# 4paradigm/OpenEmbedding

Hardware: NVIDIA H100
Metric: samples/sec (whole job, device-timed, max over ranks) deepfm Criteo dim 64 (higher is better)
Workload: dtype bf16

## Files before the change

openembedding_b200/csrc/cuda/gemm_wgmma.cu:

```cuda
#include <cuda.h>
#include <cuda_bf16.h>
#include <cuda_runtime.h>
#include "pdl.cuh"
#include <stdint.h>
#include <stdio.h>
#include <stdlib.h>
#include <string.h>

#include <string>
#include <vector>
#include <algorithm>

namespace {

constexpr int BM = 128, BK = 64;
constexpr int A_BYTES = BM * BK * 2;
template <int BN> constexpr int stages_for() { return BN == 64 ? 4 : 3; }
constexpr int NUM_CONSUMER_WARPS = 8;
constexpr int PRODUCER_WARP = NUM_CONSUMER_WARPS;
constexpr int NUM_THREADS = 32 * (NUM_CONSUMER_WARPS + 1);

enum EpiMode : int { EPI_FWD = 0, EPI_DX = 1, EPI_DW = 2, EPI_DX_FM = 3 };

struct GemmEpi {
// ... 34 lines not shown
    for (uint32_t it = 0; it < (1u << 24); ++it)
        if (mbar_try(b, parity)) return true;
    atomicAdd(&g_pipeline_timeouts, 1u);
    return false;
}
__device__ __forceinline__ void tma_load_2d(void* smem_dst, const CUtensorMap* map, uint64_t* bar, int c0, int c1) {
    asm volatile("cp.async.bulk.tensor.2d.shared::cluster.global.mbarrier::complete_tx::bytes [%0], [%1, {%3, %4}], [%2];"
                 ::"r"(smem_u32(smem_dst)), "l"(map), "r"(smem_u32(bar)), "r"(c0), "r"(c1) : "memory");
}
__device__ __forceinline__ void tma_load_2d_mc(void* smem_dst, const CUtensorMap* map, uint64_t* bar, int c0, int c1, uint16_t mask) {
    asm volatile("cp.async.bulk.tensor.2d.shared::cluster.global.mbarrier::complete_tx::bytes.multicast::cluster [%0], [%1, {%4, %5}], [%2], %3;"
                 ::"r"(smem_u32(smem_dst)), "l"(map), "r"(smem_u32(bar)), "h"(mask), "r"(c0), "r"(c1) : "memory");
}
__device__ __forceinline__ void cluster_sync_all() {
    asm volatile("barrier.cluster.arrive.release.aligned;" ::: "memory");
    asm volatile("barrier.cluster.wait.acquire.aligned;" ::: "memory");
}
__device__ __forceinline__ void named_bar_sync(int id, int threads) {
    asm volatile("bar.sync %0, %1;" ::"r"(id), "r"(threads) : "memory");
}

__device__ __forceinline__ uint64_t gmma_desc(uint32_t smem_addr, uint32_t lbo_bytes) {
    uint64_t d = 0;
    d |= (uint64_t)((smem_addr & 0x3FFFFu) >> 4);
    d |= (uint64_t)((lbo_bytes >> 4) & 0x3FFFu) << 16;
    d |= (uint64_t)(1024 >> 4) << 32;
    d |= (uint64_t)1 << 62;
    return d;
}
__device__ __forceinline__ void wgmma_fence() { asm volatile("wgmma.fence.sync.aligned;" ::: "memory"); }
__device__ __forceinline__ void wgmma_commit() { asm volatile("wgmma.commit_group.sync.aligned;" ::: "memory"); }
template <int N>
__device__ __forceinline__ void wgmma_wait() { asm volatile("wgmma.wait_group.sync.aligned %0;" ::"n"(N) : "memory"); }
template <int R>
__device__ __forceinline__ void acc_fence(float (&d)[R]) {
#pragma unroll
    for (int i = 0; i < R; ++i) asm volatile("" : "+f"(d[i])::"memory");
}

template <int TRANS>
__device__ __forceinline__ void wgmma_n64(float (&d)[32], uint64_t da, uint64_t db, uint32_t scale_d) {
    asm volatile("{\n\t.reg .pred p;\n\tsetp.ne.b32 p, %34, 0;\n\t"
                 "wgmma.mma_async.sync.aligned.m64n64k16.f32.bf16.bf16 {"
                 "%0, %1, %2, %3, %4, %5, %6, %7, %8, %9, %10, %11, %12, %13, %14, %15, "
                 "%16, %17, %18, %19, %20, %21, %22, %23, %24, %25, %26, %27, %28, %29, %30, %31"
                 "}, %32, %33, p, 1, 1, %35, %35;\n\t}"
                 : "+f"(d[0]), "+f"(d[1]), "+f"(d[2]), "+f"(d[3]), "+f"(d[4]), "+f"(d[5]), "+f"(d[6]), "+f"(d[7]),
                   "+f"(d[8]), "+f"(d[9]), "+f"(d[10]), "+f"(d[11]), "+f"(d[12]), "+f"(d[13]), "+f"(d[14]), "+f"(d[15]),
                   "+f"(d[16]), "+f"(d[17]), "+f"(d[18]), "+f"(d[19]), "+f"(d[20]), "+f"(d[21]), "+f"(d[22]), "+f"(d[23]),
                   "+f"(d[24]), "+f"(d[25]), "+f"(d[26]), "+f"(d[27]), "+f"(d[28]), "+f"(d[29]), "+f"(d[30]), "+f"(d[31])
                 : "l"(da), "l"(db), "r"(scale_d), "n"(TRANS));
}
template <int TRANS>
__device__ __forceinline__ void wgmma_n128(float (&d)[64], uint64_t da, uint64_t db, uint32_t scale_d) {
    asm volatile("{\n\t.reg .pred p;\n\tsetp.ne.b32 p, %66, 0;\n\t"
                 "wgmma.mma_async.sync.aligned.m64n128k16.f32.bf16.bf16 {"
                 "%0, %1, %2, %3, %4, %5, %6, %7, %8, %9, %10, %11, %12, %13, %14, %15, "
                 "%16, %17, %18, %19, %20, %21, %22, %23, %24, %25, %26, %27, %28, %29, %30, %31, "
                 "%32, %33, %34, %35, %36, %37, %38, %39, %40, %41, %42, %43, %44, %45, %46, %47, "
                 "%48, %49, %50, %51, %52, %53, %54, %55, %56, %57, %58, %59, %60, %61, %62, %63"
                 "}, %64, %65, p, 1, 1, %67, %67;\n\t}"
                 : "+f"(d[0]), "+f"(d[1]), "+f"(d[2]), "+f"(d[3]), "+f"(d[4]), "+f"(d[5]), "+f"(d[6]), "+f"(d[7]),
                   "+f"(d[8]), "+f"(d[9]), "+f"(d[10]), "+f"(d[11]), "+f"(d[12]), "+f"(d[13]), "+f"(d[14]), "+f"(d[15]),
                   "+f"(d[16]), "+f"(d[17]), "+f"(d[18]), "+f"(d[19]), "+f"(d[20]), "+f"(d[21]), "+f"(d[22]), "+f"(d[23]),
                   "+f"(d[24]), "+f"(d[25]), "+f"(d[26]), "+f"(d[27]), "+f"(d[28]), "+f"(d[29]), "+f"(d[30]), "+f"(d[31]),
                   "+f"(d[32]), "+f"(d[33]), "+f"(d[34]), "+f"(d[35]), "+f"(d[36]), "+f"(d[37]), "+f"(d[38]), "+f"(d[39]),
                   "+f"(d[40]), "+f"(d[41]), "+f"(d[42]), "+f"(d[43]), "+f"(d[44]), "+f"(d[45]), "+f"(d[46]), "+f"(d[47]),
                   "+f"(d[48]), "+f"(d[49]), "+f"(d[50]), "+f"(d[51]), "+f"(d[52]), "+f"(d[53]), "+f"(d[54]), "+f"(d[55]),
                   "+f"(d[56]), "+f"(d[57]), "+f"(d[58]), "+f"(d[59]), "+f"(d[60]), "+f"(d[61]), "+f"(d[62]), "+f"(d[63])
                 : "l"(da), "l"(db), "r"(scale_d), "n"(TRANS));
}
template <int BN, int TRANS>
__device__ __forceinline__ void wgmma_stage(float (&acc)[BN / 2], uint32_t a0, uint32_t b0, int g, bool first) {
#pragma unroll
    for (int k = 0; k < BK / 16; ++k) {
        const uint64_t da = TRANS ? gmma_desc(a0 + g * 8192 + k * 2048, 8192) : gmma_desc(a0 + g * 8192 + k * 32, 16);
        const uint64_t db = TRANS ? gmma_desc(b0 + k * 2048, 8192) : gmma_desc(b0 + k * 32, 16);
        const uint32_t sd = (first && k == 0) ? 0u : 1u;
        if constexpr (BN == 64) wgmma_n64<TRANS>(acc, da, db, sd);
        else wgmma_n128<TRANS>(acc, da, db, sd);
    }
}

template <int BN>
__device__ __forceinline__ void mma_tile(float (&acc)[BN / 2], const uint8_t* sA, const uint8_t* sB, uint64_t* full,
                                         uint64_t* empty, int stages, uint32_t kiter, int nkb, bool mn_major, int g,
                                         int C) {
    constexpr int B_BYTES = BN * BK * 2;
    const int lane = threadIdx.x & 31;
#pragma unroll
    for (int j = 0; j < BN / 2; ++j) acc[j] = 0.f;
    auto release = [&](uint32_t it) {
        const int s = it % stages;
        if (C > 1) { if (lane < C) mbar_arrive_cluster(&empty[s], (uint32_t)lane); }
        else if (lane == 0) mbar_arrive(&empty[s]);
    };
    for (int i = 0; i < nkb; ++i) {
        const uint32_t it = kiter + i;
        const int s = it % stages;
        mbar_wait(&full[s], (it / stages) & 1u);
        const uint32_t a0 = smem_u32(sA + s * A_BYTES), b0 = smem_u32(sB + s * B_BYTES);
        wgmma_fence();
        if (mn_major) wgmma_stage<BN, 1>(acc, a0, b0, g, i == 0);
        else wgmma_stage<BN, 0>(acc, a0, b0, g, i == 0);
        wgmma_commit();
        if (i > 0) {
            wgmma_wait<1>();
            acc_fence(acc);
            release(it - 1);
        }
    }
    wgmma_wait<0>();
    acc_fence(acc);
    if (nkb > 0) release(kiter + nkb - 1);
}

template <int BN>
__device__ __forceinline__ void epilogue_tile(const GemmEpi& E, float (&acc)[BN / 2], int m_blk, int n_blk, int g,
                                              uint8_t* stage, int qstride, const CUtensorMap* tO, const CUtensorMap* tT) {
    const int t = threadIdx.x & 127, w = t >> 5, l = t & 31;
    const bool f32out = (E.mode == EPI_DW || E.mode == EPI_DX_FM);
    const int q = 2 * g + (w >> 1);
    uint8_t* wstage = stage + q * qstride;
    uint8_t* tstage = wstage + BN * 128;
#pragma unroll
    for (int i = 0; i < 2; ++i) {
        const int qrow = (w & 1) * 16 + (l >> 2) + 8 * i;
        const int row = m_blk * BM + q * 32 + qrow;
        const bool rv = row < E.M;
        const float dl = (E.mode == EPI_DX_FM && rv && n_blk * BN < E.fm_cols) ? E.dlogit[row] : 0.f;
#pragma unroll
        for (int j = 0; j < BN / 8; ++j) {
            const int c = 8 * j + 2 * (l & 3);
            const int n = n_blk * BN + c;
            float x[2] = {acc[4 * j + 2 * i], acc[4 * j + 2 * i + 1]};
            if (E.mode == EPI_FWD) {
#pragma unroll
                for (int u = 0; u < 2; ++u) {
                    if (E.relu) x[u] = fmaxf(x[u], 0.f);
                    if (n + u == E.ones_col) x[u] = 1.f;
                    if (n + u >= E.N) x[u] = 0.f;
                }
            } else if (E.mode == EPI_DX) {
                float2 mk = make_float2(0.f, 0.f);
                if (rv && n < E.N) mk = __bfloat1622float2(*reinterpret_cast<const __nv_bfloat162*>(E.mask + (size_t)row * E.ldmask + n));
                const float mv[2] = {mk.x, mk.y};
#pragma unroll
                for (int u = 0; u < 2; ++u)
                    if (!rv || !(mv[u] > 0.f) || n + u == E.ones_col || n + u >= E.N) x[u] = 0.f;
            } else if (E.mode == EPI_DX_FM && rv && n < E.fm_cols) {
                const float2 e2 = *reinterpret_cast<const float2*>(E.emb + (size_t)row * E.ldemb + n);
                const float* sb = E.S + (size_t)row * E.D;
                x[0] += dl * (sb[n % E.D] - e2.x);
                x[1] += dl * (sb[(n + 1) % E.D] - e2.y);
            }
            if (f32out) {
                const int cc = c & 31;
                *reinterpret_cast<float2*>(wstage + (c >> 5) * 4096 + qrow * 128 + ((((cc >> 2) ^ (qrow & 7))) << 4) + (cc & 3) * 4) =
                    make_float2(x[0], x[1]);
            } else {
                const int cc = c & 63;
                *reinterpret_cast<__nv_bfloat162*>(wstage + (c >> 6) * 4096 + qrow * 128 + ((((cc >> 3) ^ (qrow & 7))) << 4) + (cc & 7) * 2) =
                    __floats2bfloat162_rn(x[0], x[1]);
                if (E.outT) {
                    *reinterpret_cast<__nv_bfloat16*>(tstage + c * 64 + qrow * 2) = __float2bfloat16_rn(x[0]);
                    *reinterpret_cast<__nv_bfloat16*>(tstage + (c + 1) * 64 + qrow * 2) = __float2bfloat16_rn(x[1]);
                }
            }
        }
    }
    asm volatile("fence.proxy.async.shared::cta;" ::: "memory");
    named_bar_sync(2 + g, 128);
    if (t == 0) {
        if (E.fm_cols != -7) {
#pragma unroll 1
            for (int qq = 2 * g; qq < 2 * g + 2; ++qq) {
                const int row0 = m_blk * BM + qq * 32;
                uint8_t* ws = stage + qq * qstride;
                if (f32out) {
#pragma unroll 1
                    for (int h = 0; h < BN / 32; ++h) {
                        const int n0 = n_blk * BN + 32 * h;
                        if (E.mode == EPI_DW)
                            asm volatile("cp.reduce.async.bulk.tensor.2d.global.shared::cta.add.tile.bulk_group [%0, {%2, %3}], [%1];"
                                         ::"l"(tO), "r"(smem_u32(ws + h * 4096)), "r"(n0), "r"(row0) : "memory");
                        else
                            asm volatile("cp.async.bulk.tensor.2d.global.shared::cta.bulk_group [%0, {%2, %3}], [%1];"
                                         ::"l"(tO), "r"(smem_u32(ws + h * 4096)), "r"(n0), "r"(row0) : "memory");
                    }
                } else {
#pragma unroll 1
                    for (int h = 0; h < BN / 64; ++h)
                        asm volatile("cp.async.bulk.tensor.2d.global.shared::cta.bulk_group [%0, {%2, %3}], [%1];"
                                     ::"l"(tO), "r"(smem_u32(ws + h * 4096)), "r"(n_blk * BN + 64 * h), "r"(row0) : "memory");
                    if (E.outT)
                        asm volatile("cp.async.bulk.tensor.2d.global.shared::cta.bulk_group [%0, {%2, %3}], [%1];"
                                     ::"l"(tT), "r"(smem_u32(ws + BN * 128)), "r"(row0), "r"(n_blk * BN) : "memory");
                }
            }
        }
        asm volatile("cp.async.bulk.commit_group;" ::: "memory");
    }
}

template <int BN>
__global__ void __launch_bounds__(NUM_THREADS, 2)
exb_gemm_wgmma_kernel(const __grid_constant__ CUtensorMap tmA, const __grid_constant__ CUtensorMap tmB,
                      const __grid_constant__ CUtensorMap tmO, const __grid_constant__ CUtensorMap tmT,
                      GemmEpi E, int num_k_blocks, int k_blocks_per_split) {
    static_assert(BN == 64 || BN == 128, "tile width");
    constexpr int STAGES = stages_for<BN>();
    constexpr int B_BYTES = BN * BK * 2;
    constexpr int QSTAGE = BN * 128 + BN * 64;
    static_assert(4 * QSTAGE <= STAGES * (A_BYTES + B_BYTES), "epilogue staging aliases the stage memory");
    extern __shared__ __align__(1024) uint8_t smem_raw[];
    uint8_t* smem = smem_raw + ((1024u - (smem_u32(smem_raw) & 1023u)) & 1023u);
    uint8_t* sA = smem;
    uint8_t* sB = smem + STAGES * A_BYTES;
    uint64_t* full = reinterpret_cast<uint64_t*>(sB + STAGES * B_BYTES);
    uint64_t* empty = full + STAGES;

    exb::pdl_trigger();
    const int warp = threadIdx.x >> 5, lane = threadIdx.x & 31;
    const int m_blk = E.swap ? blockIdx.y : blockIdx.x, n_blk = E.swap ? blockIdx.x : blockIdx.y;
    const bool dbg = E.dbg != nullptr && blockIdx.x == 0 && blockIdx.y == 0 && blockIdx.z == 0;
#define GSTAMP(i) do { if (dbg) { unsigned long long _t; asm volatile("mov.u64 %0, %%globaltimer;" : "=l"(_t)); E.dbg[i] = _t; } } while (0)
    if (threadIdx.x == 0) GSTAMP(0);
    const int kb0 = blockIdx.z * k_blocks_per_split;
    const int kb1 = min(num_k_blocks, kb0 + k_blocks_per_split);
    const int nkb = kb1 - kb0;
    const int C = E.mc > 1 ? E.mc : 1;
    uint32_t crank = 0;
    if (C > 1) asm volatile("mov.u32 %0, %%cluster_ctarank;" : "=r"(crank));
    const uint16_t cmask = (uint16_t)((1u << C) - 1u);

    if (threadIdx.x == 0) {
        for (int i = 0; i < STAGES; ++i) { mbar_init(&full[i], 1); mbar_init(&empty[i], (uint32_t)(NUM_CONSUMER_WARPS * C)); }
        asm volatile("fence.mbarrier_init.release.cluster;" ::: "memory");
        asm volatile("prefetch.tensormap [%0];" ::"l"(&tmA) : "memory");
        asm volatile("prefetch.tensormap [%0];" ::"l"(&tmB) : "memory");
    }
    __syncthreads();
    if (C > 1) cluster_sync_all();
    exb::pdl_wait();
    if (threadIdx.x == 0) GSTAMP(1);

    if (warp == PRODUCER_WARP) {
        if (lane == 0) {
            for (int i = 0; i < nkb; ++i) {
                const int s = i % STAGES;
                const uint32_t ph = (uint32_t)(i / STAGES) & 1u;
                mbar_wait(&empty[s], ph ^ 1u);
                mbar_expect_tx(&full[s], A_BYTES + B_BYTES);
                if (E.mn_major) {
                    if (C > 1) {
                        if (crank == 0) {
                            tma_load_2d_mc(sA + s * A_BYTES, &tmA, &full[s], m_blk * BM, (kb0 + i) * BK, cmask);
                            tma_load_2d_mc(sA + s * A_BYTES + A_BYTES / 2, &tmA, &full[s], m_blk * BM + 64, (kb0 + i) * BK, cmask);
                        }
                    } else {
                        tma_load_2d(sA + s * A_BYTES, &tmA, &full[s], m_blk * BM, (kb0 + i) * BK);
                        tma_load_2d(sA + s * A_BYTES + A_BYTES / 2, &tmA, &full[s], m_blk * BM + 64, (kb0 + i) * BK);
                    }
#pragma unroll
                    for (int h = 0; h < BN / 64; ++h)
                        tma_load_2d(sB + s * B_BYTES + h * 8192, &tmB, &full[s], n_blk * BN + 64 * h, (kb0 + i) * BK);
                    continue;
                }
                if (C > 1) {
                    if (crank == 0) tma_load_2d_mc(sA + s * A_BYTES, &tmA, &full[s], (kb0 + i) * BK, m_blk * BM, cmask);
                } else {
                    tma_load_2d(sA + s * A_BYTES, &tmA, &full[s], (kb0 + i) * BK, m_blk * BM);
                }
                tma_load_2d(sB + s * B_BYTES, &tmB, &full[s], (kb0 + i) * BK, n_blk * BN);
            }
        }
    } else {
        const int g = warp >> 2;
        float acc[BN / 2];
        if (dbg && threadIdx.x == 0 && nkb > 0) { mbar_wait(&full[0], 0); GSTAMP(2); }
        mma_tile<BN>(acc, sA, sB, full, empty, STAGES, 0u, nkb, E.mn_major != 0, g, C);
        if (threadIdx.x == 0) GSTAMP(3);
        named_bar_sync(1, 32 * NUM_CONSUMER_WARPS);
        epilogue_tile<BN>(E, acc, m_blk, n_blk, g, smem, QSTAGE, &tmO, &tmT);
        if ((threadIdx.x & 127) == 0) asm volatile("cp.async.bulk.wait_group.read 0;" ::: "memory");
        if (threadIdx.x == 0) GSTAMP(4);
    }
    __syncthreads();
    if (threadIdx.x == 0) GSTAMP(5);
    if (C > 1) cluster_sync_all();
}

constexpr int CH_STAGES = 3;
constexpr int CH_BN = 64;
constexpr int CH_B_BYTES = CH_BN * BK * 2;
constexpr int CH_MAX_PROB = 8;
constexpr int CH_MAX_MB = 64;

struct ChainMaps { CUtensorMap tmA, tmB, tmO; };
struct ChainMapsAll { ChainMaps m[CH_MAX_PROB]; };
struct ChainMeta {
    GemmEpi E;
    int m_tiles, n_tiles, splits, nkb, per;
    int item0, items;
    int dep, dep_kind, dep_need;
    int signal;
};

__device__ __forceinline__ void ch_decode(const ChainMeta* M, int nprob, int item, int& p, int& m, int& n, int& z) {
    p = 0;
#pragma unroll 1
    for (int i = 1; i < nprob; ++i)
        if (item >= M[i].item0) p = i;
    const int local = item - M[p].item0;
    const int mn = M[p].m_tiles * M[p].n_tiles;
    z = local / mn;
    const int r = local - z * mn;
    m = r / M[p].n_tiles;
    n = r - m * M[p].n_tiles;
}
__device__ __forceinline__ unsigned ch_ld_acquire(const unsigned* p) {
    unsigned v;
    asm volatile("ld.acquire.gpu.global.u32 %0, [%1];" : "=r"(v) : "l"(p) : "memory");
    return v;
}

__global__ void __launch_bounds__(NUM_THREADS, 2)
exb_gemm_chain_kernel(const __grid_constant__ ChainMapsAll MAPS, const ChainMeta* __restrict__ metas, int nprob, int total_items,
                      unsigned* __restrict__ ready, int* __restrict__ err) {
    const ChainMaps* maps = MAPS.m;
    extern __shared__ __align__(1024) uint8_t smem_raw[];
    uint8_t* smem = smem_raw + ((1024u - (smem_u32(smem_raw) & 1023u)) & 1023u);
    uint8_t* sA = smem;
    uint8_t* sB = smem + CH_STAGES * A_BYTES;
    uint8_t* sStage = sB + CH_STAGES * CH_B_BYTES;
    uint64_t* full = reinterpret_cast<uint64_t*>(sStage + 4 * 8192);
    uint64_t* empty = full + CH_STAGES;
    ChainMeta* M = reinterpret_cast<ChainMeta*>(empty + CH_STAGES);

    exb::pdl_trigger();
    const int warp = threadIdx.x >> 5, lane = threadIdx.x & 31;
    for (int i = threadIdx.x; i < nprob * (int)(sizeof(ChainMeta) / 4); i += blockDim.x)
        reinterpret_cast<uint32_t*>(M)[i] = reinterpret_cast<const uint32_t*>(metas)[i];
    if (threadIdx.x == 0) {
        for (int i = 0; i < CH_STAGES; ++i) { mbar_init(&full[i], 1); mbar_init(&empty[i], NUM_CONSUMER_WARPS); }
        asm volatile("fence.mbarrier_init.release.cluster;" ::: "memory");
    }
    __syncthreads();
    exb::pdl_wait();

    if (warp == PRODUCER_WARP) {
        if (lane == 0) {
            uint32_t kiter = 0;
            for (int item = blockIdx.x; item < total_items; item += gridDim.x) {
                int p, m_blk, n_blk, z;
                ch_decode(M, nprob, item, p, m_blk, n_blk, z);
                const ChainMeta& Q = M[p];
                const int kb0 = z * Q.per, kb1 = min(Q.nkb, kb0 + Q.per);
                if (Q.dep_kind) {
                    int mb0 = m_blk, mb1 = m_blk + 1;
                    if (Q.dep_kind == 2) { mb0 = (kb0 * BK) / BM; mb1 = (kb1 * BK + BM - 1) / BM; }
                    const unsigned* cnt = ready + Q.dep * CH_MAX_MB;
                    for (int mb = mb0; mb < mb1; ++mb) {
                        uint32_t it = 0;
                        while (ch_ld_acquire(cnt + mb) < (unsigned)Q.dep_need) {
                            __nanosleep(64);
                            if (++it > (1u << 22)) { atomicCAS(err, 0, 100 + p); break; }
                        }
                    }
                    asm volatile("fence.proxy.async;" ::: "memory");
                }
                const CUtensorMap* tA = &maps[p].tmA;
                const CUtensorMap* tB = &maps[p].tmB;
                for (int kb = kb0; kb < kb1; ++kb, ++kiter) {
                    const int s = kiter % CH_STAGES;
                    const uint32_t ph = (kiter / CH_STAGES) & 1u;
                    mbar_wait(&empty[s], ph ^ 1u);
                    mbar_expect_tx(&full[s], A_BYTES + CH_B_BYTES);
                    if (Q.E.mn_major) {
                        tma_load_2d(sA + s * A_BYTES, tA, &full[s], m_blk * BM, kb * BK);
                        tma_load_2d(sA + s * A_BYTES + A_BYTES / 2, tA, &full[s], m_blk * BM + 64, kb * BK);
                        tma_load_2d(sB + s * CH_B_BYTES, tB, &full[s], n_blk * CH_BN, kb * BK);
                    } else {
                        tma_load_2d(sA + s * A_BYTES, tA, &full[s], kb * BK, m_blk * BM);
                        tma_load_2d(sB + s * CH_B_BYTES, tB, &full[s], kb * BK, n_blk * CH_BN);
                    }
                }
            }
        }
    } else {
        const int g = warp >> 2;
        uint32_t kiter = 0;
        float acc[CH_BN / 2];
        for (int item = blockIdx.x; item < total_items; item += gridDim.x) {
            int p, m_blk, n_blk, z;
            ch_decode(M, nprob, item, p, m_blk, n_blk, z);
            const ChainMeta& Q = M[p];
            const int kb0 = z * Q.per, kb1 = min(Q.nkb, kb0 + Q.per);
            const int nk = __shfl_sync(0xffffffffu, kb1 - kb0, 0);
            const int mn = __shfl_sync(0xffffffffu, Q.E.mn_major, 0);
            mma_tile<CH_BN>(acc, sA, sB, full, empty, CH_STAGES, kiter, nk, mn != 0, g, 1);
            kiter += nk;
            epilogue_tile<CH_BN>(Q.E, acc, m_blk, n_blk, g, sStage, 8192, &maps[p].tmO, &maps[p].tmO);
            if ((threadIdx.x & 127) == 0) {
                if (Q.signal) {
                    asm volatile("cp.async.bulk.wait_group 0;" ::: "memory");
                    asm volatile("fence.proxy.async;" ::: "memory");
                    __threadfence();
                    atomicAdd(&ready[p * CH_MAX_MB + m_blk], 1u);
                } else {
                    asm volatile("cp.async.bulk.wait_group.read 0;" ::: "memory");
                }
            }
            named_bar_sync(2 + g, 128);
        }
    }
    __syncthreads();
    if (warp == 0) {
        unsigned last = 0;
        if (lane == 0) {
            __threadfence();
            last = (atomicAdd(&ready[CH_MAX_PROB * CH_MAX_MB], 1u) == gridDim.x - 1) ? 1u : 0u;
        }
        last = __shfl_sync(0xffffffffu, last, 0);
        if (last) {
            for (int i = lane; i < CH_MAX_PROB * CH_MAX_MB; i += 32) ready[i] = 0u;
            __syncwarp();
            if (lane == 0) { __threadfence(); ready[CH_MAX_PROB * CH_MAX_MB] = 0u; }
        }
    }
}

typedef CUresult (*EncodeTiledFn)(CUtensorMap*, CUtensorMapDataType, cuuint32_t, void*, const cuuint64_t*,
                                  const cuuint64_t*, const cuuint32_t*, const cuuint32_t*, CUtensorMapInterleave,
                                  CUtensorMapSwizzle, CUtensorMapL2promotion, CUtensorMapFloatOOBfill);
EncodeTiledFn g_encode = nullptr;
thread_local std::string g_gemm_err;

bool make_map_ex(CUtensorMap* map, CUtensorMapDataType dt, int esize, const void* ptr, long long rows, long long cols,
                 long long ld, int box_cols, int box_rows, CUtensorMapSwizzle sw);

bool make_map(CUtensorMap* map, const void* ptr, long long rows, long long cols, long long ld, int box_rows) {
    return make_map_ex(map, CU_TENSOR_MAP_DATA_TYPE_BFLOAT16, 2, ptr, rows, cols, ld, BK, box_rows, CU_TENSOR_MAP_SWIZZLE_128B);
}

bool make_map_ex(CUtensorMap* map, CUtensorMapDataType dt, int esize, const void* ptr, long long rows, long long cols,
                 long long ld, int box_cols, int box_rows, CUtensorMapSwizzle sw) {
    if (!g_encode) {
        void* fn = nullptr;
        cudaDriverEntryPointQueryResult qres;
        if (cudaGetDriverEntryPoint("cuTensorMapEncodeTiled", &fn, cudaEnableDefault, &qres) != cudaSuccess || !fn) {
            g_gemm_err = "cuTensorMapEncodeTiled entry point not found";
            return false;
        }
        g_encode = (EncodeTiledFn)fn;
    }
    cuuint64_t dims[2] = {(cuuint64_t)cols, (cuuint64_t)rows};
    cuuint64_t strides[1] = {(cuuint64_t)ld * esize};
    cuuint32_t box[2] = {(cuuint32_t)box_cols, (cuuint32_t)box_rows};
    cuuint32_t estr[2] = {1, 1};
    CUresult r = g_encode(map, dt, 2, const_cast<void*>(ptr), dims, strides, box, estr,
                          CU_TENSOR_MAP_INTERLEAVE_NONE, sw, CU_TENSOR_MAP_L2_PROMOTION_L2_128B,
                          CU_TENSOR_MAP_FLOAT_OOB_FILL_NONE);
    if (r != CUDA_SUCCESS) {
        g_gemm_err = "cuTensorMapEncodeTiled failed: " + std::to_string((int)r);
        return false;
    }
    return true;
}

template <int BN>
constexpr size_t gemm_smem() { return stages_for<BN>() * (A_BYTES + BN * BK * 2) + (2 * stages_for<BN>() + 1) * 8 + 16 + 1024; }

int pick_swap() {
    static int v = -1;
    if (v < 0) { const char* e = getenv("EXB_GEMM_SWAP"); v = e ? atoi(e) : 0; }
    return v;
}
int pick_bn(int M, int N, int K) {
    static int forced = -1;
    if (forced < 0) { const char* e = getenv("EXB_GEMM_BN"); forced = e ? atoi(e) : 0; }
    if (forced == 64 || forced == 128) return forced;
    if (K <= 128 && N >= 512 && M >= 8192) return 128;
    return 64;
}

template <int BN>
cudaError_t launch_gemm(dim3 grid, cudaStream_t stream, const CUtensorMap& tmA, const CUtensorMap& tmB, const CUtensorMap& tmO,
                        const CUtensorMap& tmT, const GemmEpi& E, int nkb, int per) {
    static bool attr_set = false;
    if (!attr_set) {
        cudaFuncSetAttribute(exb_gemm_wgmma_kernel<BN>, cudaFuncAttributeMaxDynamicSharedMemorySize, (int)gemm_smem<BN>());
        attr_set = true;
    }
    if (E.mc > 1) {
        cudaLaunchConfig_t cfg = {};
        cfg.gridDim = grid; cfg.blockDim = dim3(NUM_THREADS); cfg.dynamicSmemBytes = gemm_smem<BN>(); cfg.stream = stream;
        cudaLaunchAttribute attr[2];
// ... 82 lines not shown
    memset(&E, 0, sizeof(E));
    E.mode = EPI_DW; E.ones_col = -1; E.M = M; E.N = N; E.D = 1; E.mn_major = 1;
    E.out = (void*)out; E.ldo = ldo;
    const int BN = pick_bn(M, N, K);
    const int nkb = K / BK;
    if (splits < 1) splits = 1;
    if (splits > nkb) splits = nkb;
    const int per = (nkb + splits - 1) / splits;
    splits = (nkb + per - 1) / per;
    dim3 grid((M + BM - 1) / BM, (N + BN - 1) / BN, splits);
    E.swap = pick_swap(); E.mc = pick_mc((int)grid.y);
    if (E.swap) grid = dim3(grid.y, grid.x, grid.z);
    cudaError_t err = BN == 128 ? launch_gemm<128>(grid, (cudaStream_t)stream, tmA, tmB, tmO, tmT, E, nkb, per)
                                : launch_gemm<64>(grid, (cudaStream_t)stream, tmA, tmB, tmO, tmT, E, nkb, per);
    if (err == cudaSuccess) err = cudaGetLastError();
    if (err != cudaSuccess) { g_gemm_err = std::string("gemm_tn launch: ") + cudaGetErrorString(err); return -1; }
    return 0;
}

struct ChainDesc {
    int tn;
    int M, N, K;
    unsigned long long A, B, out;
    long long lda, ldb, ldo;
    int mode, relu, ones_col, fm_cols, D, splits;
    unsigned long long mask; long long ldmask;
    unsigned long long dlogit, S, emb; long long ldemb;
    int dep, dep_kind;
};
struct Chain {
    int nprob = 0, total = 0, grid = 0;
    ChainMapsAll maps;
    ChainMeta* d_meta = nullptr;
    unsigned* d_ready = nullptr;
    int* d_err = nullptr;
    size_t smem = 0;
};

int exb_chain_desc_size() { return (int)sizeof(ChainDesc); }

void* exb_chain_create(const void* descs, int n, int sms) {
    if (n < 1 || n > CH_MAX_PROB) { g_gemm_err = "chain: 1..8 GEMMs"; return nullptr; }
    const ChainDesc* D = reinterpret_cast<const ChainDesc*>(descs);
    std::vector<ChainMaps> maps(n);
    std::vector<ChainMeta> meta(n);
    int item0 = 0;
    for (int i = 0; i < n; ++i) {
        const ChainDesc& d = D[i];
        ChainMeta& Q = meta[i];
        memset(&Q, 0, sizeof(Q));
        if (d.K % BK != 0 || d.lda % 8 != 0 || d.ldb % 8 != 0) { g_gemm_err = "chain: K % 64 / ld % 8 violated"; return nullptr; }
        GemmEpi& E = Q.E;
        E.mode = d.tn ? EPI_DW : d.mode; E.relu = d.relu; E.ones_col = d.tn ? -1 : d.ones_col; E.fm_cols = d.fm_cols;
        E.M = d.M; E.N = d.N; E.D = d.D > 0 ? d.D : 1; E.mn_major = d.tn ? 1 : 0;
        E.out = (void*)d.out; E.ldo = d.ldo; E.outT = nullptr; E.ldoT = 0;
        E.mask = (const __nv_bfloat16*)d.mask; E.ldmask = d.ldmask;
        E.dlogit = (const float*)d.dlogit; E.S = (const float*)d.S; E.emb = (const float*)d.emb; E.ldemb = d.ldemb;
        E.swap = 0; E.mc = 1; E.dbg = nullptr;
        const bool f32out = (E.mode == EPI_DW || E.mode == EPI_DX_FM);
        bool ok;
        if (d.tn) {
            ok = make_map_ex(&maps[i].tmA, CU_TENSOR_MAP_DATA_TYPE_BFLOAT16, 2, (const void*)d.A, d.K, d.M, d.lda, 64, BK, CU_TENSOR_MAP_SWIZZLE_128B) &&
                 make_map_ex(&maps[i].tmB, CU_TENSOR_MAP_DATA_TYPE_BFLOAT16, 2, (const void*)d.B, d.K, d.N, d.ldb, 64, BK, CU_TENSOR_MAP_SWIZZLE_128B);
        } else {
            ok = make_map(&maps[i].tmA, (const void*)d.A, d.M, d.K, d.lda, BM) && make_map(&maps[i].tmB, (const void*)d.B, d.N, d.K, d.ldb, CH_BN);
        }
        if (ok) {
            if (f32out) ok = make_map_ex(&maps[i].tmO, CU_TENSOR_MAP_DATA_TYPE_FLOAT32, 4, (const void*)d.out, d.M, d.N, d.ldo, 32, 32, CU_TENSOR_MAP_SWIZZLE_128B);
            else ok = make_map_ex(&maps[i].tmO, CU_TENSOR_MAP_DATA_TYPE_BFLOAT16, 2, (const void*)d.out, d.M, (d.N + 63) / 64 * 64, d.ldo, 64, 32, CU_TENSOR_MAP_SWIZZLE_128B);
        }
        if (!ok) return nullptr;
        Q.nkb = d.K / BK;
        int splits = d.tn ? std::max(1, d.splits) : 1;
        if (splits > Q.nkb) splits = Q.nkb;
        Q.per = (Q.nkb + splits - 1) / splits;
        Q.splits = (Q.nkb + Q.per - 1) / Q.per;
        Q.m_tiles = (d.M + BM - 1) / BM; Q.n_tiles = (d.N + CH_BN - 1) / CH_BN;
        Q.item0 = item0; Q.items = Q.m_tiles * Q.n_tiles * Q.splits;
        item0 += Q.items;
        Q.dep = d.dep; Q.dep_kind = d.dep >= 0 ? d.dep_kind : 0; Q.dep_need = 0; Q.signal = 0;
        if (Q.dep_kind) {
            if (d.dep >= i) { g_gemm_err = "chain: a GEMM may only depend on an earlier one"; return nullptr; }
            meta[d.dep].signal = 1;
            Q.dep_need = (NUM_CONSUMER_WARPS / 4) * meta[d.dep].n_tiles;
            if (meta[d.dep].m_tiles > CH_MAX_MB) { g_gemm_err = "chain: too many row blocks"; return nullptr; }
        }
    }
    Chain* c = new Chain();
    c->nprob = n; c->total = item0;
    c->smem = CH_STAGES * (A_BYTES + CH_B_BYTES) + 4 * 8192 + 2 * CH_STAGES * 8 + CH_MAX_PROB * sizeof(ChainMeta) + 1024;
    cudaFuncSetAttribute(exb_gemm_chain_kernel, cudaFuncAttributeMaxDynamicSharedMemorySize, (int)c->smem);
    cudaFuncSetAttribute(exb_gemm_chain_kernel, cudaFuncAttributePreferredSharedMemoryCarveout, 100);
    int occ = (2 * (c->smem + 1024) <= 232448) ? 2 : 1;
    if (const char* ev = getenv("EXB_CHAIN_CTAS_PER_SM")) occ = std::max(1, std::min(2, atoi(ev)));
    c->grid = std::min(c->total, (sms > 0 ? sms : 132) * occ);
    memset(&c->maps, 0, sizeof(c->maps));
    for (int i = 0; i < n; ++i) c->maps.m[i] = maps[i];
    if (cudaMalloc(&c->d_meta, n * sizeof(ChainMeta)) != cudaSuccess ||
        cudaMalloc(&c->d_ready, (CH_MAX_PROB * CH_MAX_MB + 32) * 4) != cudaSuccess || cudaMalloc(&c->d_err, 4) != cudaSuccess) {
        g_gemm_err = "chain: cudaMalloc failed"; delete c; return nullptr;
    }
    cudaMemcpy(c->d_meta, meta.data(), n * sizeof(ChainMeta), cudaMemcpyHostToDevice);
    cudaMemset(c->d_ready, 0, (CH_MAX_PROB * CH_MAX_MB + 32) * 4);
    cudaMemset(c->d_err, 0, 4);
    return c;
}
void exb_chain_destroy(void* h) {
    Chain* c = (Chain*)h;
    cudaFree(c->d_meta); cudaFree(c->d_ready); cudaFree(c->d_err);
    delete c;
}
int exb_chain_launch(void* h, uint64_t stream) {
    Chain* c = (Chain*)h;
    cudaError_t err = exb::launch_pdl(exb_gemm_chain_kernel, dim3(c->grid), dim3(NUM_THREADS), c->smem, (cudaStream_t)stream,
                              c->maps, (const ChainMeta*)c->d_meta, c->nprob, c->total, c->d_ready, c->d_err);
    if (err == cudaSuccess) err = cudaGetLastError();
    if (err != cudaSuccess) { g_gemm_err = std::string("chain launch: ") + cudaGetErrorString(err); return -1; }
    return 0;
}
int exb_chain_status(void* h) {
    Chain* c = (Chain*)h;
    int v = 0;
    cudaDeviceSynchronize();
    cudaMemcpy(&v, c->d_err, 4, cudaMemcpyDeviceToHost);
    return v;
}
int exb_chain_info(void* h, int* out) { Chain* c = (Chain*)h; out[0] = c->total; out[1] = c->grid; out[2] = (int)c->smem; return 0; }

}
```

Baseline: 12.34 million.

## Restructure chained GEMM kernel into ping-pong warpgroups with 128-wide tiles

Reworks the persistent chain GEMM kernel so two consumer warpgroups each compute a full 128x128 tile (two M-halves per warpgroup) and alternate tiles in ping-pong order, handing off via mbarriers so one group's epilogue overlaps the other's MMA. Adds setmaxnreg register rebalancing between producer and consumer warpgroups, increases pipeline stages to 4, and drops to one CTA per SM. The epilogue is specialized per mode through templates, preloads mask/embedding inputs, and streams output in column slices through double-buffered staging. It risks lower occupancy, register pressure and more complex synchronization in exchange for better overlap and larger tile reuse.

```diff
diff --git a/openembedding_b200/csrc/cuda/gemm_wgmma.cu b/openembedding_b200/csrc/cuda/gemm_wgmma.cu
--- a/openembedding_b200/csrc/cuda/gemm_wgmma.cu
+++ b/openembedding_b200/csrc/cuda/gemm_wgmma.cu
@@ -140,14 +140,16 @@
     }
 }
 
-template <int BN>
-__device__ __forceinline__ void mma_tile(float (&acc)[BN / 2], const uint8_t* sA, const uint8_t* sB, uint64_t* full,
+template <int BN, int RH>
+__device__ __forceinline__ void mma_tile(float (&acc)[RH][BN / 2], const uint8_t* sA, const uint8_t* sB, uint64_t* full,
                                          uint64_t* empty, int stages, uint32_t kiter, int nkb, bool mn_major, int g,
-                                         int C) {
+                                         int C, uint64_t* handoff = nullptr) {
     constexpr int B_BYTES = BN * BK * 2;
     const int lane = threadIdx.x & 31;
 #pragma unroll
-    for (int j = 0; j < BN / 2; ++j) acc[j] = 0.f;
+    for (int h = 0; h < RH; ++h)
+#pragma unroll
+        for (int j = 0; j < BN / 2; ++j) acc[h][j] = 0.f;
     auto release = [&](uint32_t it) {
         const int s = it % stages;
         if (C > 1) { if (lane < C) mbar_arrive_cluster(&empty[s], (uint32_t)lane); }
@@ -159,101 +161,144 @@
         mbar_wait(&full[s], (it / stages) & 1u);
         const uint32_t a0 = smem_u32(sA + s * A_BYTES), b0 = smem_u32(sB + s * B_BYTES);
         wgmma_fence();
-        if (mn_major) wgmma_stage<BN, 1>(acc, a0, b0, g, i == 0);
-        else wgmma_stage<BN, 0>(acc, a0, b0, g, i == 0);
+#pragma unroll
+        for (int h = 0; h < RH; ++h) {
+            if (mn_major) wgmma_stage<BN, 1>(acc[h], a0, b0, g + h, i == 0);
+            else wgmma_stage<BN, 0>(acc[h], a0, b0, g + h, i == 0);
+        }
         wgmma_commit();
         if (i > 0) {
             wgmma_wait<1>();
-            acc_fence(acc);
+#pragma unroll
+            for (int h = 0; h < RH; ++h) acc_fence(acc[h]);
             release(it - 1);
         }
     }
+    if (handoff) mbar_arrive(handoff);
     wgmma_wait<0>();
-    acc_fence(acc);
+#pragma unroll
+    for (int h = 0; h < RH; ++h) acc_fence(acc[h]);
     if (nkb > 0) release(kiter + nkb - 1);
 }
 
-template <int BN>
-__device__ __forceinline__ void epilogue_tile(const GemmEpi& E, float (&acc)[BN / 2], int m_blk, int n_blk, int g,
-                                              uint8_t* stage, int qstride, const CUtensorMap* tO, const CUtensorMap* tT) {
+struct EpiIn { float2 a, b; };
+__device__ __forceinline__ EpiIn epi_load(const GemmEpi& E, const int mode, int row, int n, bool rv, bool fm) {
+    EpiIn in = {make_float2(0.f, 0.f), make_float2(0.f, 0.f)};
+    if (mode == EPI_DX) {
+        const size_t off = (rv && n < E.N) ? (size_t)row * E.ldmask + n : 0;
+        in.a = __bfloat1622float2(__ldg(reinterpret_cast<const __nv_bfloat162*>(E.mask + off)));
+    } else if (mode == EPI_DX_FM && fm) {
+        const bool ok = rv && n < E.fm_cols;
+        const size_t r = ok ? row : 0;
+        const int c = ok ? n : 0;
+        in.a = __ldg(reinterpret_cast<const float2*>(E.emb + r * E.ldemb + c));
+        const float* sb = E.S + r * E.D;
+        const int nd = c % E.D, nd1 = nd + 1 == E.D ? 0 : nd + 1;
+        in.b = make_float2(__ldg(sb + nd), __ldg(sb + nd1));
+    }
+    return in;
+}
+
+__device__ __forceinline__ void epi_pair(const GemmEpi& E, const int mode, float (&x)[2], const EpiIn& in, int n, bool rv,
+                                         bool fm, float dl) {
+    if (mode == EPI_FWD) {
+#pragma unroll
+        for (int u = 0; u < 2; ++u) {
+            if (E.relu) x[u] = fmaxf(x[u], 0.f);
+            if (n + u == E.ones_col) x[u] = 1.f;
+            if (n + u >= E.N) x[u] = 0.f;
+        }
+    } else if (mode == EPI_DX) {
+        const float mv[2] = {in.a.x, in.a.y};
+#pragma unroll
+        for (int u = 0; u < 2; ++u)
+            if (!rv || !(mv[u] > 0.f) || n + u == E.ones_col || n + u >= E.N) x[u] = 0.f;
+    } else if (mode == EPI_DX_FM && fm && rv && n < E.fm_cols) {
+        x[0] += dl * (in.b.x - in.a.x);
+        x[1] += dl * (in.b.y - in.a.y);
+    }
+}
+
+template <int BN, int RH, int MODE, int C0, int CW, bool PRELOAD>
+__device__ __forceinline__ void epilogue_tile(const GemmEpi& E, float (&acc)[RH][BN / 2], int row0, int col0,
+                                              uint8_t* stage, int qstride, const CUtensorMap* tO,
+                                              const CUtensorMap* tT, int bar) {
     const int t = threadIdx.x & 127, w = t >> 5, l = t & 31;
-    const bool f32out = (E.mode == EPI_DW || E.mode == EPI_DX_FM);
-    const int q = 2 * g + (w >> 1);
-    uint8_t* wstage = stage + q * qstride;
-    uint8_t* tstage = wstage + BN * 128;
-#pragma unroll
-    for (int i = 0; i < 2; ++i) {
-        const int qrow = (w & 1) * 16 + (l >> 2) + 8 * i;
-        const int row = m_blk * BM + q * 32 + qrow;
-        const bool rv = row < E.M;
-        const float dl = (E.mode == EPI_DX_FM && rv && n_blk * BN < E.fm_cols) ? E.dlogit[row] : 0.f;
-#pragma unroll
-        for (int j = 0; j < BN / 8; ++j) {
-            const int c = 8 * j + 2 * (l & 3);
-            const int n = n_blk * BN + c;
-            float x[2] = {acc[4 * j + 2 * i], acc[4 * j + 2 * i + 1]};
-            if (E.mode == EPI_FWD) {
-#pragma unroll
-                for (int u = 0; u < 2; ++u) {
-                    if (E.relu) x[u] = fmaxf(x[u], 0.f);
-                    if (n + u == E.ones_col) x[u] = 1.f;
-                    if (n + u >= E.N) x[u] = 0.f;
+    const int mode = MODE >= 0 ? MODE : E.mode;
+    const bool f32out = (mode == EPI_DW || mode == EPI_DX_FM);
+    const bool fm = mode == EPI_DX_FM && col0 < E.fm_cols;
+    auto row_of = [&](int h, int i) { return row0 + (2 * h + (w >> 1)) * 32 + (w & 1) * 16 + (l >> 2) + 8 * i; };
+#pragma unroll
+    for (int h = 0; h < RH; ++h) {
+        EpiIn in[2][BN / 8];
+        if constexpr (PRELOAD) {
+#pragma unroll
+            for (int i = 0; i < 2; ++i)
+#pragma unroll
+                for (int j = C0 / 8; j < (C0 + CW) / 8; ++j) {
+                    const int row = row_of(h, i);
+                    in[i][j] = epi_load(E, mode, row, col0 + 8 * j + 2 * (l & 3), row < E.M, fm);
                 }
-            } else if (E.mode == EPI_DX) {
-                float2 mk = make_float2(0.f, 0.f);
-                if (rv && n < E.N) mk = __bfloat1622float2(*reinterpret_cast<const __nv_bfloat162*>(E.mask + (size_t)row * E.ldmask + n));
-                const float mv[2] = {mk.x, mk.y};
-#pragma unroll
-                for (int u = 0; u < 2; ++u)
-                    if (!rv || !(mv[u] > 0.f) || n + u == E.ones_col || n + u >= E.N) x[u] = 0.f;
-            } else if (E.mode == EPI_DX_FM && rv && n < E.fm_cols) {
-                const float2 e2 = *reinterpret_cast<const float2*>(E.emb + (size_t)row * E.ldemb + n);
-                const float* sb = E.S + (size_t)row * E.D;
-                x[0] += dl * (sb[n % E.D] - e2.x);
-                x[1] += dl * (sb[(n + 1) % E.D] - e2.y);
-            }
-            if (f32out) {
-                const int cc = c & 31;
-                *reinterpret_cast<float2*>(wstage + (c >> 5) * 4096 + qrow * 128 + ((((cc >> 2) ^ (qrow & 7))) << 4) + (cc & 3) * 4) =
-                    make_float2(x[0], x[1]);
-            } else {
-                const int cc = c & 63;
-                *reinterpret_cast<__nv_bfloat162*>(wstage + (c >> 6) * 4096 + qrow * 128 + ((((cc >> 3) ^ (qrow & 7))) << 4) + (cc & 7) * 2) =
-                    __floats2bfloat162_rn(x[0], x[1]);
-                if (E.outT) {
-                    *reinterpret_cast<__nv_bfloat16*>(tstage + c * 64 + qrow * 2) = __float2bfloat16_rn(x[0]);
-                    *reinterpret_cast<__nv_bfloat16*>(tstage + (c + 1) * 64 + qrow * 2) = __float2bfloat16_rn(x[1]);
+        }
+        const int q = 2 * h + (w >> 1);
+        uint8_t* wstage = stage + q * qstride;
+        uint8_t* tstage = wstage + BN * 128;
+#pragma unroll
+        for (int i = 0; i < 2; ++i) {
+            const int qrow = (w & 1) * 16 + (l >> 2) + 8 * i;
+            const int row = row_of(h, i);
+            const bool rv = row < E.M;
+            const float dl = fm ? (rv ? __ldg(E.dlogit + row) : 0.f) : 0.f;
+#pragma unroll
+            for (int j = C0 / 8; j < (C0 + CW) / 8; ++j) {
+                const int c = 8 * j + 2 * (l & 3);
+                const int n = col0 + c;
+                if constexpr (!PRELOAD) in[i][j] = epi_load(E, mode, row, n, rv, fm);
+                float x[2] = {acc[h][4 * j + 2 * i], acc[h][4 * j + 2 * i + 1]};
+                epi_pair(E, mode, x, in[i][j], n, rv, fm, dl);
+                if (f32out) {
+                    const int cc = c & 31;
+                    *reinterpret_cast<float2*>(wstage + ((c - C0) >> 5) * 4096 + qrow * 128 + ((((cc >> 2) ^ (qrow & 7))) << 4) + (cc & 3) * 4) =
+                        make_float2(x[0], x[1]);
+                } else {
+                    const int cc = c & 63;
+                    *reinterpret_cast<__nv_bfloat162*>(wstage + ((c - C0) >> 6) * 4096 + qrow * 128 + ((((cc >> 3) ^ (qrow & 7))) << 4) + (cc & 7) * 2) =
+                        __floats2bfloat162_rn(x[0], x[1]);
+                    if (E.outT) {
+                        *reinterpret_cast<__nv_bfloat16*>(tstage + c * 64 + qrow * 2) = __float2bfloat16_rn(x[0]);
+                        *reinterpret_cast<__nv_bfloat16*>(tstage + (c + 1) * 64 + qrow * 2) = __float2bfloat16_rn(x[1]);
+                    }
                 }
             }
         }
     }
     asm volatile("fence.proxy.async.shared::cta;" ::: "memory");
-    named_bar_sync(2 + g, 128);
+    named_bar_sync(bar, 128);
     if (t == 0) {
         if (E.fm_cols != -7) {
 #pragma unroll 1
-            for (int qq = 2 * g; qq < 2 * g + 2; ++qq) {
-                const int row0 = m_blk * BM + qq * 32;
+            for (int qq = 0; qq < 2 * RH; ++qq) {
+                const int r0 = row0 + qq * 32;
                 uint8_t* ws = stage + qq * qstride;
                 if (f32out) {
 #pragma unroll 1
-                    for (int h = 0; h < BN / 32; ++h) {
-                        const int n0 = n_blk * BN + 32 * h;
-                        if (E.mode == EPI_DW)
+                    for (int h = 0; h < CW / 32; ++h) {
+                        const int n0 = col0 + C0 + 32 * h;
+                        if (mode == EPI_DW)
                             asm volatile("cp.reduce.async.bulk.tensor.2d.global.shared::cta.add.tile.bulk_group [%0, {%2, %3}], [%1];"
-                                         ::"l"(tO), "r"(smem_u32(ws + h * 4096)), "r"(n0), "r"(row0) : "memory");
+                                         ::"l"(tO), "r"(smem_u32(ws + h * 4096)), "r"(n0), "r"(r0) : "memory");
                         else
                             asm volatile("cp.async.bulk.tensor.2d.global.shared::cta.bulk_group [%0, {%2, %3}], [%1];"
-                                         ::"l"(tO), "r"(smem_u32(ws + h * 4096)), "r"(n0), "r"(row0) : "memory");
+                                         ::"l"(tO), "r"(smem_u32(ws + h * 4096)), "r"(n0), "r"(r0) : "memory");
                     }
                 } else {
 #pragma unroll 1
-                    for (int h = 0; h < BN / 64; ++h)
+                    for (int h = 0; h < CW / 64; ++h)
                         asm volatile("cp.async.bulk.tensor.2d.global.shared::cta.bulk_group [%0, {%2, %3}], [%1];"
-                                     ::"l"(tO), "r"(smem_u32(ws + h * 4096)), "r"(n_blk * BN + 64 * h), "r"(row0) : "memory");
+                                     ::"l"(tO), "r"(smem_u32(ws + h * 4096)), "r"(col0 + C0 + 64 * h), "r"(r0) : "memory");
                     if (E.outT)
                         asm volatile("cp.async.bulk.tensor.2d.global.shared::cta.bulk_group [%0, {%2, %3}], [%1];"
-                                     ::"l"(tT), "r"(smem_u32(ws + BN * 128)), "r"(row0), "r"(n_blk * BN) : "memory");
+                                     ::"l"(tT), "r"(smem_u32(ws + BN * 128)), "r"(r0), "r"(col0) : "memory");
                 }
             }
         }
@@ -335,12 +380,21 @@
         }
     } else {
         const int g = warp >> 2;
-        float acc[BN / 2];
+        float acc[1][BN / 2];
         if (dbg && threadIdx.x == 0 && nkb > 0) { mbar_wait(&full[0], 0); GSTAMP(2); }
-        mma_tile<BN>(acc, sA, sB, full, empty, STAGES, 0u, nkb, E.mn_major != 0, g, C);
+        mma_tile<BN, 1>(acc, sA, sB, full, empty, STAGES, 0u, nkb, E.mn_major != 0, g, C);
         if (threadIdx.x == 0) GSTAMP(3);
         named_bar_sync(1, 32 * NUM_CONSUMER_WARPS);
-        epilogue_tile<BN>(E, acc, m_blk, n_blk, g, smem, QSTAGE, &tmO, &tmT);
+        const int row0 = m_blk * BM + 64 * g, col0 = n_blk * BN;
+        uint8_t* qs = smem + 2 * g * QSTAGE;
+        if constexpr (BN == 128) {
+            epilogue_tile<BN, 1, -1, 0, BN, false>(E, acc, row0, col0, qs, QSTAGE, &tmO, &tmT, 2 + g);
+        } else {
+            if (E.mode == EPI_FWD) epilogue_tile<BN, 1, EPI_FWD, 0, BN, false>(E, acc, row0, col0, qs, QSTAGE, &tmO, &tmT, 2 + g);
+            else if (E.mode == EPI_DX) epilogue_tile<BN, 1, EPI_DX, 0, BN, false>(E, acc, row0, col0, qs, QSTAGE, &tmO, &tmT, 2 + g);
+            else if (E.mode == EPI_DW) epilogue_tile<BN, 1, EPI_DW, 0, BN, false>(E, acc, row0, col0, qs, QSTAGE, &tmO, &tmT, 2 + g);
+            else epilogue_tile<BN, 1, EPI_DX_FM, 0, BN, false>(E, acc, row0, col0, qs, QSTAGE, &tmO, &tmT, 2 + g);
+        }
         if ((threadIdx.x & 127) == 0) asm volatile("cp.async.bulk.wait_group.read 0;" ::: "memory");
         if (threadIdx.x == 0) GSTAMP(4);
     }
@@ -349,9 +403,11 @@
     if (C > 1) cluster_sync_all();
 }
 
-constexpr int CH_STAGES = 3;
-constexpr int CH_BN = 64;
+constexpr int CH_STAGES = 4;
+constexpr int CH_BN = 128;
 constexpr int CH_B_BYTES = CH_BN * BK * 2;
+constexpr int CH_THREADS = 384;
+constexpr int CH_SLICE = 4 * 4096;
 constexpr int CH_MAX_PROB = 8;
 constexpr int CH_MAX_MB = 64;
 
@@ -383,7 +439,29 @@
     return v;
 }
 
-__global__ void __launch_bounds__(NUM_THREADS, 2)
+template <int MODE, int S = 0>
+__device__ __forceinline__ void chain_epilogue(const GemmEpi& E, float (&acc)[2][CH_BN / 2], int m_blk, int n_blk,
+                                               uint8_t* stage, const CUtensorMap* tO, int g) {
+    constexpr int CW = (MODE == EPI_DW || MODE == EPI_DX_FM) ? 32 : 64;
+    if constexpr (S * CW < CH_BN) {
+        if (n_blk * CH_BN + S * CW >= E.N) return;
+        if ((threadIdx.x & 127) == 0) {
+            if (S == 0) asm volatile("cp.async.bulk.wait_group.read 0;" ::: "memory");
+            else asm volatile("cp.async.bulk.wait_group.read 1;" ::: "memory");
+        }
+        named_bar_sync(2 + g, 128);
+        epilogue_tile<CH_BN, 2, MODE, S * CW, CW, true>(E, acc, m_blk * BM, n_blk * CH_BN, stage + (S & 1) * CH_SLICE, 4096,
+                                                  tO, tO, 2 + g);
+        chain_epilogue<MODE, S + 1>(E, acc, m_blk, n_blk, stage, tO, g);
+    }
+}
+
+constexpr size_t chain_smem() {
+    return CH_STAGES * (A_BYTES + CH_B_BYTES) + 2 * 2 * CH_SLICE + (2 * CH_STAGES + 2) * 8 + CH_MAX_PROB * sizeof(ChainMeta) + 1024;
+}
+static_assert(chain_smem() <= 232448, "chain shared memory exceeds the 227 KB an H100 CTA can have");
+
+__global__ void __launch_bounds__(CH_THREADS, 1)
 exb_gemm_chain_kernel(const __grid_constant__ ChainMapsAll MAPS, const ChainMeta* __restrict__ metas, int nprob, int total_items,
                       unsigned* __restrict__ ready, int* __restrict__ err) {
     const ChainMaps* maps = MAPS.m;
@@ -391,24 +469,27 @@
     uint8_t* smem = smem_raw + ((1024u - (smem_u32(smem_raw) & 1023u)) & 1023u);
     uint8_t* sA = smem;
     uint8_t* sB = smem + CH_STAGES * A_BYTES;
-    uint8_t* sStage = sB + CH_STAGES * CH_B_BYTES;
-    uint64_t* full = reinterpret_cast<uint64_t*>(sStage + 4 * 8192);
+    uint8_t* sEpi = sB + CH_STAGES * CH_B_BYTES;
+    uint64_t* full = reinterpret_cast<uint64_t*>(sEpi + 2 * 2 * CH_SLICE);
     uint64_t* empty = full + CH_STAGES;
-    ChainMeta* M = reinterpret_cast<ChainMeta*>(empty + CH_STAGES);
+    uint64_t* order = empty + CH_STAGES;
+    ChainMeta* M = reinterpret_cast<ChainMeta*>(order + 2);
 
     exb::pdl_trigger();
     const int warp = threadIdx.x >> 5, lane = threadIdx.x & 31;
     for (int i = threadIdx.x; i < nprob * (int)(sizeof(ChainMeta) / 4); i += blockDim.x)
         reinterpret_cast<uint32_t*>(M)[i] = reinterpret_cast<const uint32_t*>(metas)[i];
     if (threadIdx.x == 0) {
-        for (int i = 0; i < CH_STAGES; ++i) { mbar_init(&full[i], 1); mbar_init(&empty[i], NUM_CONSUMER_WARPS); }
+        for (int i = 0; i < CH_STAGES; ++i) { mbar_init(&full[i], 1); mbar_init(&empty[i], 4); }
+        for (int i = 0; i < 2; ++i) mbar_init(&order[i], 128);
         asm volatile("fence.mbarrier_init.release.cluster;" ::: "memory");
     }
     __syncthreads();
     exb::pdl_wait();
 
-    if (warp == PRODUCER_WARP) {
-        if (lane == 0) {
+    if (warp < 4) {
+        asm volatile("setmaxnreg.dec.sync.aligned.u32 40;" ::: "memory");
+        if (warp == 0 && lane == 0) {
             uint32_t kiter = 0;
             for (int item = blockIdx.x; item < total_items; item += gridDim.x) {
                 int p, m_blk, n_blk, z;
@@ -439,6 +520,7 @@
                         tma_load_2d(sA + s * A_BYTES, tA, &full[s], m_blk * BM, kb * BK);
                         tma_load_2d(sA + s * A_BYTES + A_BYTES / 2, tA, &full[s], m_blk * BM + 64, kb * BK);
                         tma_load_2d(sB + s * CH_B_BYTES, tB, &full[s], n_blk * CH_BN, kb * BK);
+                        tma_load_2d(sB + s * CH_B_BYTES + CH_B_BYTES / 2, tB, &full[s], n_blk * CH_BN + 64, kb * BK);
                     } else {
                         tma_load_2d(sA + s * A_BYTES, tA, &full[s], kb * BK, m_blk * BM);
                         tma_load_2d(sB + s * CH_B_BYTES, tB, &full[s], kb * BK, n_blk * CH_BN);
@@ -447,31 +529,39 @@
             }
         }
     } else {
-        const int g = warp >> 2;
+        asm volatile("setmaxnreg.inc.sync.aligned.u32 232;" ::: "memory");
+        const int g = (warp >> 2) - 1, t = threadIdx.x & 127;
+        uint8_t* stage = sEpi + g * 2 * CH_SLICE;
         uint32_t kiter = 0;
-        float acc[CH_BN / 2];
-        for (int item = blockIdx.x; item < total_items; item += gridDim.x) {
+        float acc[2][CH_BN / 2];
+        for (int local = 0; blockIdx.x + local * gridDim.x < (unsigned)total_items; ++local) {
+            const int item = blockIdx.x + local * gridDim.x;
             int p, m_blk, n_blk, z;
             ch_decode(M, nprob, item, p, m_blk, n_blk, z);
             const ChainMeta& Q = M[p];
             const int kb0 = z * Q.per, kb1 = min(Q.nkb, kb0 + Q.per);
             const int nk = __shfl_sync(0xffffffffu, kb1 - kb0, 0);
             const int mn = __shfl_sync(0xffffffffu, Q.E.mn_major, 0);
-            mma_tile<CH_BN>(acc, sA, sB, full, empty, CH_STAGES, kiter, nk, mn != 0, g, 1);
+            if ((local & 1) != g) { kiter += nk; continue; }
+            if (local > 0) mbar_wait(&order[g], (uint32_t)((local - 1) >> 1) & 1u);
+            mma_tile<CH_BN, 2>(acc, sA, sB, full, empty, CH_STAGES, kiter, nk, mn != 0, 0, 1, &order[g ^ 1]);
             kiter += nk;
-            epilogue_tile<CH_BN>(Q.E, acc, m_blk, n_blk, g, sStage, 8192, &maps[p].tmO, &maps[p].tmO);
-            if ((threadIdx.x & 127) == 0) {
-                if (Q.signal) {
-                    asm volatile("cp.async.bulk.wait_group 0;" ::: "memory");
-                    asm volatile("fence.proxy.async;" ::: "memory");
-                    __threadfence();
-                    atomicAdd(&ready[p * CH_MAX_MB + m_blk], 1u);
-                } else {
-                    asm volatile("cp.async.bulk.wait_group.read 0;" ::: "memory");
-                }
+            const GemmEpi E = Q.E;
+            const int mode = __shfl_sync(0xffffffffu, E.mode, 0);
+            const CUtensorMap* tO = &maps[p].tmO;
+            if (mode == EPI_FWD) chain_epilogue<EPI_FWD>(E, acc, m_blk, n_blk, stage, tO, g);
+            else if (mode == EPI_DX) chain_epilogue<EPI_DX>(E, acc, m_blk, n_blk, stage, tO, g);
+            else if (mode == EPI_DW) chain_epilogue<EPI_DW>(E, acc, m_blk, n_blk, stage, tO, g);
+            else chain_epilogue<EPI_DX_FM>(E, acc, m_blk, n_blk, stage, tO, g);
+            if (t == 0 && Q.signal) {
+                asm volatile("cp.async.bulk.wait_group 0;" ::: "memory");
+                asm volatile("fence.proxy.async;" ::: "memory");
+                __threadfence();
+                ch_decode(M, nprob, item, p, m_blk, n_blk, z);
+                atomicAdd(&ready[p * CH_MAX_MB + m_blk], 1u);
             }
-            named_bar_sync(2 + g, 128);
-        }
+        }
+        if (t == 0) asm volatile("cp.async.bulk.wait_group.read 0;" ::: "memory");
     }
     __syncthreads();
     if (warp == 0) {
@@ -720,18 +810,16 @@
         if (Q.dep_kind) {
             if (d.dep >= i) { g_gemm_err = "chain: a GEMM may only depend on an earlier one"; return nullptr; }
             meta[d.dep].signal = 1;
-            Q.dep_need = (NUM_CONSUMER_WARPS / 4) * meta[d.dep].n_tiles;
+            Q.dep_need = meta[d.dep].n_tiles;
             if (meta[d.dep].m_tiles > CH_MAX_MB) { g_gemm_err = "chain: too many row blocks"; return nullptr; }
         }
     }
     Chain* c = new Chain();
     c->nprob = n; c->total = item0;
-    c->smem = CH_STAGES * (A_BYTES + CH_B_BYTES) + 4 * 8192 + 2 * CH_STAGES * 8 + CH_MAX_PROB * sizeof(ChainMeta) + 1024;
+    c->smem = chain_smem();
     cudaFuncSetAttribute(exb_gemm_chain_kernel, cudaFuncAttributeMaxDynamicSharedMemorySize, (int)c->smem);
     cudaFuncSetAttribute(exb_gemm_chain_kernel, cudaFuncAttributePreferredSharedMemoryCarveout, 100);
-    int occ = (2 * (c->smem + 1024) <= 232448) ? 2 : 1;
-    if (const char* ev = getenv("EXB_CHAIN_CTAS_PER_SM")) occ = std::max(1, std::min(2, atoi(ev)));
-    c->grid = std::min(c->total, (sms > 0 ? sms : 132) * occ);
+    c->grid = std::min(c->total, sms > 0 ? sms : 132);
     memset(&c->maps, 0, sizeof(c->maps));
     for (int i = 0; i < n; ++i) c->maps.m[i] = maps[i];
     if (cudaMalloc(&c->d_meta, n * sizeof(ChainMeta)) != cudaSuccess ||
@@ -750,7 +838,7 @@
 }
 int exb_chain_launch(void* h, uint64_t stream) {
     Chain* c = (Chain*)h;
-    cudaError_t err = exb::launch_pdl(exb_gemm_chain_kernel, dim3(c->grid), dim3(NUM_THREADS), c->smem, (cudaStream_t)stream,
+    cudaError_t err = exb::launch_pdl(exb_gemm_chain_kernel, dim3(c->grid), dim3(CH_THREADS), c->smem, (cudaStream_t)stream,
                               c->maps, (const ChainMeta*)c->d_meta, c->nprob, c->total, c->d_ready, c->d_err);
     if (err == cudaSuccess) err = cudaGetLastError();
     if (err != cudaSuccess) { g_gemm_err = std::string("chain launch: ") + cudaGetErrorString(err); return -1; }
```

After: 12.66 million (median of 6 runs). +2.6%, better.
